# SvenGronauer/distributedTensorFlow

Hardware: AMD Instinct MI355X
Metric: images/sec (whole node) ResNet-50 synthetic ImageNet at 1/2/4/8 MI355X (higher is better)
Workload: dtype bf16; 1 GPU; model=resnet50, global_batch=1984, per_gpu_batch=1984, image_size=224, parallelism=dp1, impl=dtf, optimizer=momentum0.9+wd1e-4, lr 0.1*B/256 warmup500+cosine, backend=auto, native_ext=distributedtensorflow_amd/_lib/_dtf_hip.cpython-310-x86_64-linux-gnu.so

## Files before the change

### csrc/kernels/bindings.cpp

```cpp
#include <hip/hip_runtime.h>
#include <pybind11/pybind11.h>
#include <pybind11/stl.h>

#include <algorithm>
#include <stdexcept>
#include <string>
#include <vector>

#include "launch.h"

namespace py = pybind11;

namespace dlp {
struct Device { int32_t device_type; int32_t device_id; };
struct DataType { uint8_t code; uint8_t bits; uint16_t lanes; };
struct Tensor { void* data; Device device; int32_t ndim; DataType dtype; int64_t* shape;
                int64_t* strides; uint64_t byte_offset; };
struct Managed { Tensor t; void* ctx; void (*deleter)(Managed*); };
constexpr int32_t kROCM = 10;
struct Ctx { int64_t shape[1]; int64_t strides[1]; uintptr_t ptr; int device; bool opened; };
void deleter(Managed* m) {
  auto* c = static_cast<Ctx*>(m->ctx);
  if (c->opened) dtf_ipc_close(c->ptr, c->device);
  else dtf_ipc_free(c->ptr, c->device);
// ... 652 lines not shown
    check_launch("gemm_stream_bnb_dual");
  });
  m.def("gemm_set_group", &dtf_gemm_set_group);
  m.def("wgrad_get_pipe", &dtf_wgrad_get_pipe);
  m.def("lds_probe", [](int bytes, int blocks, uintptr_t errors, int spin, uintptr_t st) {
    dtf_lds_probe(bytes, blocks, P<int>(errors), spin, S(st));
    check_launch("lds_probe");
  });
  m.def("max_dynamic_lds", &dtf_max_dynamic_lds);

  m.def("ln_fwd", [](uintptr_t a, uintptr_t bias, uintptr_t res, uintptr_t gamma, uintptr_t beta,
                     uintptr_t y, uintptr_t s, uintptr_t mean, uintptr_t rstd, int M, int H,
                     float eps, float p_pre, uint32_t seed_pre, float p_post, uint32_t seed_post,
                     uintptr_t ids, uintptr_t tt, uintptr_t word, uintptr_t pos, uintptr_t type,
                     int S_, uintptr_t st) {
    dtf_ln_fwd(P<const bf16_t>(a), P<const float>(bias), P<const bf16_t>(res),
               P<const float>(gamma), P<const float>(beta), P<bf16_t>(y), P<bf16_t>(s),
               P<float>(mean), P<float>(rstd), M, H, eps, p_pre, seed_pre, p_post, seed_post,
               P<const int64_t>(ids), P<const int64_t>(tt), P<const bf16_t>(word),
               P<const bf16_t>(pos), P<const bf16_t>(type), S_, S(st));
    check_launch("ln_fwd");
  });
  m.def("ln_bwd_blocks", &dtf_ln_bwd_blocks);
  m.def("ln_bwd", [](uintptr_t dy, uintptr_t s, uintptr_t mean, uintptr_t rstd, uintptr_t gamma,
                     uintptr_t ds, uintptr_t da, uintptr_t part, uintptr_t dgamma,
                     uintptr_t dbeta, uintptr_t dbias, int M, int H, float p_pre,
                     uint32_t seed_pre, float p_post, uint32_t seed_post, uintptr_t st,
                     int accumulate) {
    dtf_ln_bwd(P<const bf16_t>(dy), P<const bf16_t>(s), P<const float>(mean),
               P<const float>(rstd), P<const float>(gamma), P<bf16_t>(ds), P<bf16_t>(da),
               P<float>(part), P<float>(dgamma), P<float>(dbeta), P<float>(dbias), M, H, p_pre,
               seed_pre, p_post, seed_post, S(st), accumulate);
    check_launch("ln_bwd");
  }, py::arg("dy"), py::arg("s"), py::arg("mean"), py::arg("rstd"), py::arg("gamma"),
     py::arg("ds"), py::arg("da"), py::arg("part"), py::arg("dgamma"), py::arg("dbeta"),
     py::arg("dbias"), py::arg("M"), py::arg("H"), py::arg("p_pre"), py::arg("seed_pre"),
     py::arg("p_post"), py::arg("seed_post"), py::arg("stream"), py::arg("accumulate") = 0);
  m.def("bias_gelu_fwd", [](uintptr_t a, uintptr_t bias, uintptr_t y, long M, int N,
                            uintptr_t st) {
    dtf_bias_gelu_fwd(P<const bf16_t>(a), P<const float>(bias), P<bf16_t>(y), M, N, S(st));
    check_launch("bias_gelu_fwd");
  });
  m.def("bias_gelu_bwd_blocks", &dtf_bias_gelu_bwd_blocks);
  m.def("bf16_col_sum_ws_floats", &dtf_bf16_col_sum_ws_floats);
  m.def("bf16_col_sum", [](uintptr_t x, int T, int N, uintptr_t ws, uintptr_t out, int accumulate,
                           uintptr_t stream) {
    dtf_bf16_col_sum(P<const bf16_t>(x), T, N, P<float>(ws), P<float>(out), accumulate, S(stream));
  });
  m.def("ln_set_wide", &dtf_ln_set_wide);
  m.def("conv1x1_bwd_ok", &dtf_conv1x1_bwd_ok);
  m.def("conv1x1_bwd_blocks", &dtf_conv1x1_bwd_blocks);
  m.def("conv1x1_bwd_set_grid", &dtf_conv1x1_bwd_set_grid);
  m.def("conv1x1_bwd_set_w16", &dtf_conv1x1_bwd_set_w16);
  m.def("conv1x1_bwd_lazy_ok", &dtf_conv1x1_bwd_lazy_ok);
  m.def("conv1x1_bwd_lazy_blocks", &dtf_conv1x1_bwd_lazy_blocks);
  m.def("conv1x1_bwd_lazy", [](uintptr_t dy3, uintptr_t x3, uintptr_t mask, uintptr_t cA,
                               uintptr_t cB, uintptr_t cC, uintptr_t wt, uintptr_t y, uintptr_t x,
                               uintptr_t mean, uintptr_t inv, uintptr_t sc, uintptr_t sh,
                               uintptr_t dy, uintptr_t wpart, uintptr_t bpart, int M, int C, int K,
                               uintptr_t w, uintptr_t stream) {
    dtf_conv1x1_bwd_lazy(P<bf16_t>(dy3), P<bf16_t>(x3), P<uint8_t>(mask), P<float>(cA),
                         P<float>(cB), P<float>(cC), P<bf16_t>(wt), P<bf16_t>(y), P<bf16_t>(x),
                         P<float>(mean), P<float>(inv), P<float>(sc), P<float>(sh), P<bf16_t>(dy),
                         P<float>(wpart), P<float>(bpart), M, C, K, P<bf16_t>(w), S(stream));
    check_launch("conv1x1_bwd_lazy");
  });
  m.def("conv1x1_bwd", [](uintptr_t dout, uintptr_t wt, uintptr_t y, uintptr_t x, uintptr_t mean,
                          uintptr_t inv, uintptr_t sc, uintptr_t sh, uintptr_t dy, uintptr_t wpart,
                          uintptr_t bpart, int M, int C, int K, uintptr_t stream) {
    dtf_conv1x1_bwd(P<bf16_t>(dout), P<bf16_t>(wt), P<bf16_t>(y), P<bf16_t>(x), P<float>(mean),
                    P<float>(inv), P<float>(sc), P<float>(sh), P<bf16_t>(dy), P<float>(wpart),
                    P<float>(bpart), M, C, K, S(stream));
    check_launch("conv1x1_bwd");
  });
  m.def("slab_reduce", [](uintptr_t ws, uintptr_t out, long n, int nsplit, int accumulate,
                          uintptr_t stream) {
    dtf_slab_reduce(P<const float>(ws), P<float>(out), n, nsplit, accumulate, S(stream));
  });
  m.def("bias_gelu_bwd", [](uintptr_t dy, uintptr_t a, uintptr_t bias, uintptr_t da,
                            uintptr_t part, uintptr_t dbias, int M, int N, uintptr_t st,
                            int accumulate) {
    dtf_bias_gelu_bwd(P<const bf16_t>(dy), P<const bf16_t>(a), P<const float>(bias),
                      P<bf16_t>(da), P<float>(part), P<float>(dbias), M, N, S(st), accumulate);
    check_launch("bias_gelu_bwd");
  }, py::arg("dy"), py::arg("a"), py::arg("bias"), py::arg("da"), py::arg("part"),
     py::arg("dbias"), py::arg("M"), py::arg("N"), py::arg("stream"), py::arg("accumulate") = 0);
  m.def("attn_fwd", [](uintptr_t qkv, uintptr_t mask, uintptr_t out, uintptr_t lse, int B, int S_,
                       int H, float scale, float p, uint32_t seed, uintptr_t st, uintptr_t keep) {
    dtf_attn_fwd(P<const bf16_t>(qkv), P<const float>(mask), P<bf16_t>(out), P<float>(lse), B,
                 S_, H, scale, p, seed, S(st), P<uint32_t>(keep));
    check_launch("attn_fwd");
  }, py::arg("qkv"), py::arg("mask"), py::arg("out"), py::arg("lse"), py::arg("B"), py::arg("S"),
     py::arg("H"), py::arg("scale"), py::arg("p"), py::arg("seed"), py::arg("st"),
     py::arg("keep") = 0);
  m.def("attn_keep_words", &dtf_attn_keep_words);
  m.def("attn_set_keep", &dtf_attn_set_keep);
  m.def("attn_bwd", [](uintptr_t qkv, uintptr_t mask, uintptr_t out, uintptr_t dout,
                       uintptr_t lse, uintptr_t delta, uintptr_t dqkv, int B, int S_, int H,
                       float scale, float p, uint32_t seed, uintptr_t st, uintptr_t colpart,
                       uintptr_t keep) {
    dtf_attn_bwd(P<const bf16_t>(qkv), P<const float>(mask), P<const bf16_t>(out),
                 P<const bf16_t>(dout), P<const float>(lse), P<float>(delta), P<bf16_t>(dqkv), B,
                 S_, H, scale, p, seed, S(st), P<float>(colpart), P<const uint32_t>(keep));
    check_launch("attn_bwd");
  }, py::arg("qkv"), py::arg("mask"), py::arg("out"), py::arg("dout"), py::arg("lse"),
     py::arg("delta"), py::arg("dqkv"), py::arg("B"), py::arg("S"), py::arg("H"),
// ... 38 lines not shown
```

### csrc/kernels/conv1x1_bwd.hip

```cpp
#include <stdexcept>
#include <string>

#include "launch.h"

namespace {

constexpr int kNB = 3;

typedef __attribute__((ext_vector_type(4))) short s4_t;
typedef __attribute__((address_space(3))) s4_t lds_s4_t;

template <int C_, int K_, int TM_, int NW_, bool LZ_ = false, bool RC_ = false>
struct Cfg {
  static constexpr int C = C_, K = K_, TM = TM_, NW = NW_;
  static constexpr bool LZ = LZ_, RC = RC_;
  static constexpr int T = NW * 64;
  static constexpr int NCB = C / 16;
  static constexpr int CPW = NCB >= NW ? NCB / NW : 1;
  static constexpr int WPC = NW / (NCB / CPW);
  static constexpr int MBW = TM / 16 / WPC;
  static constexpr int KS = K / 32;
  static constexpr int KBW = K / NW / 16;
  static constexpr int DO = TM * K;
  static constexpr int YT = TM * C;
  static constexpr int OT = (LZ && !RC) ? 2 * DO : DO;
  static constexpr int MB = LZ ? TM * K / 8 : 0;
  static constexpr int MI = MB / 1024;
  static constexpr int SLOT = OT + 2 * YT + MB / 2;
  static constexpr int DOI = OT * 2 / 1024;
  static constexpr int YI = YT * 2 / 1024;
  static constexpr int D = (DOI + 2 * YI) / NW;
  static constexpr int S = CPW * MBW;
  static constexpr int MCH = LZ ? TM * K / 8 / T : 0;
  static constexpr size_t LDS = (size_t)kNB * SLOT * 2 + (size_t)WPC * 2 * C * 4 + 4 * C * 4 +
                                (LZ ? (size_t)3 * K * 4 : 0);
  static_assert(!LZ || ((RC || ((TM * K / 8) % T == 0 && T % (K / 8) == 0)) && MB % 1024 == 0 &&
                        MI <= NW), "LZ transform split");
  static_assert(DOI % NW == 0 && (2 * YI) % NW == 0, "DMA split");
  static_assert(WPC * (NCB / CPW) == NW && MBW >= 1 && (TM % 32 == 0 || TM == 16), "wave split");
  static_assert(LDS <= 160 * 1024, "conv1x1_bwd LDS");
};

DTF_DEV int swz_o(int r) { return 2 * (r & 7) + ((r >> 3) & 1); }
template <int C>
DTF_DEV int swz_y(int r) { return C == 64 ? 2 * ((r >> 1) & 3) : 2 * (r & 7); }
template <int C>
DTF_DEV int swz_x(int r) { return C == 64 ? (r >> 1) & 7 : r & 15; }

template <int RP>
DTF_DEV int sidx(int r, int c, int s) { return r * RP + (((c >> 3) ^ s) << 3) + (c & 7); }

template <int RP, int C, bool DOUT>
DTF_DEV bf16x8_t tr8(const bf16_t* base, int row0, int col0, int lane) {
  const int i = lane & 15, g = lane >> 4;
  const int r = row0 + 4 * g + (i >> 2), c = col0 + 4 * (i & 3);
  const int s0 = DOUT ? swz_o(r) : swz_y<C>(r);
  const int s1 = DOUT ? swz_o(r + 16) : swz_y<C>(r + 16);
  const s4_t lo = __builtin_amdgcn_ds_read_tr16_b64_v4i16((lds_s4_t*)(base + sidx<RP>(r, c, s0)));
  const s4_t hi = __builtin_amdgcn_ds_read_tr16_b64_v4i16((lds_s4_t*)(base + sidx<RP>(r + 16, c, s1)));
  return (bf16x8_t){lo[0], lo[1], lo[2], lo[3], hi[0], hi[1], hi[2], hi[3]};
}

template <int RP, int C, bool DOUT>
DTF_DEV s4_t tr4(const bf16_t* base, int col0, int lane) {
  const int i = lane & 15, g = lane >> 4;
  const int r = 4 * g + (i >> 2), c = col0 + 4 * (i & 3);
  const int s0 = DOUT ? swz_o(r) : swz_y<C>(r);
  return __builtin_amdgcn_ds_read_tr16_b64_v4i16((lds_s4_t*)(base + sidx<RP>(r, c, s0)));
}

DTF_DEV f32x4_t mfma16(const bf16x8_t& a, const bf16x8_t& b, const f32x4_t& c) {
  return __builtin_amdgcn_mfma_f32_16x16x32_bf16(a, b, c, 0, 0, 0);
}

template <class F>
constexpr int RC_KBW() { return F::RC ? F::K / F::NW / 16 : 1; }

struct C1Args {
  const bf16_t* dout;
  const bf16_t* wt;
  const bf16_t* y;
  const bf16_t* x;
  const float* mean;
  const float* inv;
  const float* sc;
  const float* sh;
  bf16_t* dy;
  float* wpart;
  float* bpart;
  int M;
  const bf16_t* x3;
  const uint8_t* mask;
  const float* cA;
  const float* cB;
  const float* cC;
  const bf16_t* w;
};

template <class F>
__global__ void __launch_bounds__(F::T, 1) conv1x1_bwd_kernel(const C1Args g) {
  constexpr int C = F::C, K = F::K, TM = F::TM, NW = F::NW;
  constexpr int CPW = F::CPW, MBW = F::MBW, KS = F::KS, KBW = F::KBW, NCB = F::NCB;
  constexpr bool LZ = F::LZ;
  extern __shared__ __attribute__((aligned(16))) bf16_t lds[];
  float* sred = reinterpret_cast<float*>(lds + kNB * F::SLOT);
  float* sprm = sred + F::WPC * 2 * C;
  float* scoef = sprm + 4 * C;
  const int tid = threadIdx.x, lane = tid & 63;
  const int wave = __builtin_amdgcn_readfirstlane(tid >> 6);
  const int li = lane & 15, gq = lane >> 4;
  const int ntiles = g.M / TM;
  const int nmy = (ntiles - (int)blockIdx.x + (int)gridDim.x - 1) / (int)gridDim.x;
  const int cg = wave % (NCB / CPW), mw = wave / (NCB / CPW);

  bf16x8_t wf[CPW][KS];
#pragma unroll
  for (int j = 0; j < CPW; ++j)
#pragma unroll
    for (int ks = 0; ks < KS; ++ks)
      wf[j][ks] = *reinterpret_cast<const bf16x8_t*>(g.wt + ((cg * CPW + j) * 16 + li) * K +
                                                      ks * 32 + gq * 8);
  for (int t = tid; t < C; t += F::T) {
    sprm[t] = g.mean[t];
    sprm[C + t] = g.inv[t];
    sprm[2 * C + t] = g.sc[t];
    sprm[3 * C + t] = g.sh[t];
  }

  const uint32_t lds0 = lds_addr(lds);
  auto issue = [&](int i) {
    const bool live = !LZ || i < nmy;
    const long m0 = ((long)blockIdx.x + (long)(live ? i : 0) * gridDim.x) * TM;
    const i32x4_t ro = rsrc_quad(g.dout + m0 * K, (uint32_t)(F::DO * 2));
    const i32x4_t r3 = rsrc_quad(LZ ? g.x3 + m0 * K : g.dout, (uint32_t)(F::DO * 2));
    const i32x4_t ry = rsrc_quad(g.y + m0 * C, (uint32_t)(F::YT * 2));
    const i32x4_t rx = rsrc_quad(g.x + m0 * C, (uint32_t)(F::YT * 2));
    const uint32_t base = lds0 + (uint32_t)((i % kNB) * F::SLOT * 2);
    constexpr int OL = K / 8, YL = C / 8;
    constexpr int OI1 = F::DO * 2 / 1024;
#pragma unroll
    for (int j = 0; j < F::DOI / NW; ++j) {
      const int q = wave + NW * j;
      const int qq = q % OI1, e = qq * 64 + lane;
      const int r = e / OL, s = e % OL;
      const uint32_t off = live ? (uint32_t)((r * K + ((s ^ swz_o(r)) << 3)) * 2) : 0xFFFFFFF0u;
      dma16(q < OI1 ? ro : r3, base + (uint32_t)q * 1024u, off);
    }
#pragma unroll
    for (int j = 0; j < 2 * F::YI / NW; ++j) {
      const int q = wave + NW * j;
      const bool isx = q >= F::YI;
      const int qq = isx ? q - F::YI : q, e = qq * 64 + lane;
      const int r = e / YL, s = e % YL;
      const int sw = isx ? swz_x<C>(r) : swz_y<C>(r);
      const uint32_t off = live ? (uint32_t)((r * C + ((s ^ sw) << 3)) * 2) : 0xFFFFFFF0u;
      dma16(isx ? rx : ry, base + (uint32_t)(F::OT * 2 + q * 1024), off);
    }
    if constexpr (LZ) {
      if (wave < F::MI) {
        const i32x4_t rm = rsrc_quad(g.mask + m0 * (K / 8), (uint32_t)F::MB);
        dma16(rm, base + (uint32_t)((F::OT + 2 * F::YT) * 2 + wave * 1024),
              live ? (uint32_t)(wave * 1024 + lane * 16) : 0xFFFFFFF0u);
      }
    }
  };
  constexpr int MCH = F::MCH > 0 ? F::MCH : 1;
  if constexpr (LZ) {
    for (int t = tid; t < K; t += F::T) {
      scoef[t] = g.cA[t];
      scoef[K + t] = g.cB[t];
      scoef[2 * K + t] = g.cC[t];
    }
  }
  constexpr int KSC = C / 32;
  bf16x8_t wr[RC_KBW<F>()][KSC];
  float rca[RC_KBW<F>()][4], rcb[RC_KBW<F>()][4], rcc[RC_KBW<F>()][4];
  if constexpr (F::RC) {
#pragma unroll
    for (int kb = 0; kb < RC_KBW<F>(); ++kb) {
#pragma unroll
      for (int ks = 0; ks < KSC; ++ks)
        wr[kb][ks] = *reinterpret_cast<const bf16x8_t*>(
            g.w + (long)(wave * (K / NW) + kb * 16 + li) * C + ks * 32 + gq * 8);
      const int k0 = wave * (K / NW) + kb * 16 + 4 * gq;
#pragma unroll
      for (int r = 0; r < 4; ++r) {
        rca[kb][r] = g.cA[k0 + r];
        rcb[kb][r] = g.cB[k0 + r];
        rcc[kb][r] = g.cC[k0 + r];
      }
    }
  }

  f32x4_t aw[KBW][NCB];
#pragma unroll
  for (int a = 0; a < KBW; ++a)
#pragma unroll
    for (int b = 0; b < NCB; ++b) aw[a][b] = (f32x4_t){0.f, 0.f, 0.f, 0.f};
  float s1[CPW][4], s2[CPW][4];
#pragma unroll
  for (int j = 0; j < CPW; ++j)
#pragma unroll
    for (int e = 0; e < 4; ++e) s1[j][e] = s2[j][e] = 0.f;

  constexpr int D = F::D, S = F::S;
  if constexpr (LZ) {
    issue(0);
    issue(1);
  } else {
    issue(0);
    if (nmy > 1) issue(1);
  }
  for (int i = 0; i < nmy; ++i) {
    if constexpr (LZ) {
      if (wave < F::MI) {
        if (i == 0) wait_vm<D + 1>();
        else if (i == 1) wait_vm<D + 1 + S>();
        else wait_vm<D + 1 + 2 * S>();
      } else {
        if (i == 0) wait_vm<D>();
        else if (i == 1) wait_vm<D + S>();
        else wait_vm<D + 2 * S>();
      }
    } else {
      const bool more = i + 1 < nmy;
      if (i == 0) { if (more) wait_vm<D>(); else wait_vm<0>(); }
      else if (i == 1) { if (more) wait_vm<D + S>(); else wait_vm<S>(); }
      else { if (more) wait_vm<D + 2 * S>(); else wait_vm<2 * S>(); }
    }
    asm volatile("s_waitcnt lgkmcnt(0)" ::: "memory");
    raw_barrier();
    if constexpr (LZ) {
      issue(i + 2);
    } else {
      if (i + 2 < nmy) issue(i + 2);
    }
    bf16_t* const slot = lds + (i % kNB) * F::SLOT;
    if constexpr (LZ && F::RC) {
      int lx = lane;
      asm volatile("" : "+v"(lx));
      const int xi = lx & 15, xq = lx >> 4;
      const uint8_t* msk = reinterpret_cast<const uint8_t*>(slot + F::OT + 2 * F::YT);
#pragma unroll
      for (int mb = 0; mb < TM / 16; ++mb) {
        const int m = mb * 16 + xi;
        bf16x8_t yb[KSC];
#pragma unroll
        for (int ks = 0; ks < KSC; ++ks)
          yb[ks] = *reinterpret_cast<const bf16x8_t*>(slot + F::OT + sidx<C>(m, ks * 32 + xq * 8, swz_y<C>(m)));
#pragma unroll
        for (int kb = 0; kb < RC_KBW<F>(); ++kb) {
          f32x4_t a = (f32x4_t){0.f, 0.f, 0.f, 0.f};
#pragma unroll
          for (int ks = 0; ks < KSC; ++ks) a = mfma16(wr[kb][ks], yb[ks], a);
          const int k0 = wave * (K / NW) + kb * 16 + 4 * xq;
          const int o = sidx<K>(m, k0, swz_o(m));
          const uint2 d = *reinterpret_cast<const uint2*>(slot + o);
          const uint32_t mbits = (uint32_t)msk[m * (K / 8) + (k0 >> 3)] >> (k0 & 7);
          const float* ca = rca[kb];
          const float* cb = rcb[kb];
          const float* cc = rcc[kb];
          const float gv[4] = {__builtin_bit_cast(float, d.x << 16), __builtin_bit_cast(float, d.x & 0xffff0000u),
                               __builtin_bit_cast(float, d.y << 16), __builtin_bit_cast(float, d.y & 0xffff0000u)};
          float ov[4];
#pragma unroll
          for (int r = 0; r < 4; ++r) {
            const float xv = bf2f(f2bf(a[r]));
            const float dz = (mbits >> r) & 1u ? gv[r] : 0.f;
            ov[r] = bn_bwd_dx(ca[r], dz, cb[r], xv, cc[r]);
          }
          *reinterpret_cast<uint2*>(slot + o) = make_uint2(pack2(ov[0], ov[1]), pack2(ov[2], ov[3]));
        }
      }
      asm volatile("s_waitcnt lgkmcnt(0)" ::: "memory");
      raw_barrier();
    } else if constexpr (LZ) {
      int tt = tid;
      asm volatile("" : "+v"(tt));
      const int lch = tt % (K / 8), lrow = tt / (K / 8);
#pragma unroll
      for (int k = 0; k < MCH; ++k) {
        const int r = lrow + k * (F::T / (K / 8));
        const int o = sidx<K>(r, lch * 8, swz_o(r));
        float gv[8], xv[8], ov[8];
        unpack8(*reinterpret_cast<const uint4*>(slot + o), gv);
        unpack8(*reinterpret_cast<const uint4*>(slot + F::DO + o), xv);
        const uint32_t mb = reinterpret_cast<const uint8_t*>(slot + F::OT + 2 * F::YT)[r * (K / 8) + lch];
        float ca[8], cb[8], cc[8];
        *reinterpret_cast<float4*>(ca) = *reinterpret_cast<const float4*>(scoef + lch * 8);
        *reinterpret_cast<float4*>(ca + 4) = *reinterpret_cast<const float4*>(scoef + lch * 8 + 4);
        *reinterpret_cast<float4*>(cb) = *reinterpret_cast<const float4*>(scoef + K + lch * 8);
        *reinterpret_cast<float4*>(cb + 4) = *reinterpret_cast<const float4*>(scoef + K + lch * 8 + 4);
        *reinterpret_cast<float4*>(cc) = *reinterpret_cast<const float4*>(scoef + 2 * K + lch * 8);
        *reinterpret_cast<float4*>(cc + 4) = *reinterpret_cast<const float4*>(scoef + 2 * K + lch * 8 + 4);
#pragma unroll
        for (int e = 0; e < 8; ++e) {
          const float dz = (mb >> e) & 1u ? gv[e] : 0.f;
          ov[e] = bn_bwd_dx(ca[e], dz, cb[e], xv[e], cc[e]);
        }
        *reinterpret_cast<uint4*>(slot + o) = pack8(ov);
      }
      asm volatile("s_waitcnt lgkmcnt(0)" ::: "memory");
      raw_barrier();
    }
    const bf16_t* sO = slot;
    const bf16_t* sY = sO + F::OT;
    const bf16_t* sX = sY + F::YT;
    int ln = lane;
    asm volatile("" : "+v"(ln));
    const int li = ln & 15, gq = ln >> 4;

    f32x4_t ad[CPW][MBW];
#pragma unroll
    for (int j = 0; j < CPW; ++j)
#pragma unroll
      for (int f = 0; f < MBW; ++f) ad[j][f] = (f32x4_t){0.f, 0.f, 0.f, 0.f};
#pragma unroll
    for (int ks = 0; ks < KS; ++ks) {
#pragma unroll
      for (int f = 0; f < MBW; ++f) {
        const int m = (mw * MBW + f) * 16 + li;
        const bf16x8_t b = *reinterpret_cast<const bf16x8_t*>(sO + sidx<K>(m, ks * 32 + gq * 8, swz_o(m)));
#pragma unroll
        for (int j = 0; j < CPW; ++j) ad[j][f] = mfma16(wf[j][ks], b, ad[j][f]);
      }
    }
    if constexpr (TM == 16) {
      s4_t fa[KBW];
#pragma unroll
      for (int kb = 0; kb < KBW; ++kb) fa[kb] = tr4<K, C, true>(sO, wave * (K / NW) + kb * 16, ln);
#pragma unroll
      for (int cb = 0; cb < NCB; ++cb) {
        const s4_t fb = tr4<C, C, false>(sY, cb * 16, ln);
#pragma unroll
        for (int kb = 0; kb < KBW; ++kb)
          aw[kb][cb] = __builtin_amdgcn_mfma_f32_16x16x16bf16_1k(fa[kb], fb, aw[kb][cb], 0, 0, 0);
      }
    }
#pragma unroll
    for (int ms = 0; ms < TM / 32; ++ms) {
      bf16x8_t fa[KBW];
#pragma unroll
      for (int kb = 0; kb < KBW; ++kb) fa[kb] = tr8<K, C, true>(sO, 32 * ms, wave * (K / NW) + kb * 16, ln);
#pragma unroll
      for (int cb = 0; cb < NCB; ++cb) {
        const bf16x8_t fb = tr8<C, C, false>(sY, 32 * ms, cb * 16, ln);
#pragma unroll
        for (int kb = 0; kb < KBW; ++kb) aw[kb][cb] = mfma16(fa[kb], fb, aw[kb][cb]);
      }
    }
    const long m0 = ((long)blockIdx.x + (long)i * gridDim.x) * TM;
#pragma unroll
    for (int j = 0; j < CPW; ++j) {
      const int c0 = (cg * CPW + j) * 16 + 4 * gq;
      float mu[4], is[4], sc[4], sh[4];
#pragma unroll
      for (int e = 0; e < 4; ++e) {
        mu[e] = sprm[c0 + e];
        is[e] = sprm[C + c0 + e];
        sc[e] = sprm[2 * C + c0 + e];
        sh[e] = sprm[3 * C + c0 + e];
      }
#pragma unroll
      for (int f = 0; f < MBW; ++f) {
        const int m = (mw * MBW + f) * 16 + li;
        const uint2 pk = make_uint2(pack2(ad[j][f][0], ad[j][f][1]), pack2(ad[j][f][2], ad[j][f][3]));
        *reinterpret_cast<uint2*>(g.dy + (m0 + m) * C + c0) = pk;
        const uint2 xr = *reinterpret_cast<const uint2*>(sX + sidx<C>(m, c0, swz_x<C>(m)));
        const float gd[4] = {__builtin_bit_cast(float, pk.x << 16), __builtin_bit_cast(float, pk.x & 0xffff0000u),
                             __builtin_bit_cast(float, pk.y << 16), __builtin_bit_cast(float, pk.y & 0xffff0000u)};
        const float xv[4] = {__builtin_bit_cast(float, xr.x << 16), __builtin_bit_cast(float, xr.x & 0xffff0000u),
                             __builtin_bit_cast(float, xr.y << 16), __builtin_bit_cast(float, xr.y & 0xffff0000u)};
#pragma unroll
        for (int e = 0; e < 4; ++e) {
          const float dz = __builtin_fmaf(xv[e], sc[e], sh[e]) > 0.f ? gd[e] : 0.f;
          s1[j][e] += dz;
          s2[j][e] += dz * (xv[e] - mu[e]) * is[e];
        }
      }
    }
  }
  DTF_WAIT_VM(0);
  asm volatile("s_waitcnt lgkmcnt(0)" ::: "memory");
  raw_barrier();

#pragma unroll
  for (int j = 0; j < CPW; ++j)
#pragma unroll
    for (int e = 0; e < 4; ++e) {
#pragma unroll
      for (int o = 1; o < 16; o <<= 1) {
        s1[j][e] += __shfl_xor(s1[j][e], o, 64);
        s2[j][e] += __shfl_xor(s2[j][e], o, 64);
      }
    }
  if (li == 0) {
#pragma unroll
    for (int j = 0; j < CPW; ++j)
#pragma unroll
      for (int e = 0; e < 4; ++e) {
        const int c = (cg * CPW + j) * 16 + 4 * gq + e;
        sred[(mw * 2 + 0) * C + c] = s1[j][e];
        sred[(mw * 2 + 1) * C + c] = s2[j][e];
      }
  }
  __syncthreads();
  for (int t = tid; t < 2 * C; t += F::T) {
    const int which = t / C, col = t % C;
    float v = 0.f;
#pragma unroll
    for (int w = 0; w < F::WPC; ++w) v += sred[(w * 2 + which) * C + col];
    g.bpart[((long)blockIdx.x * 2 + which) * C + col] = v;
  }
  float* wp = g.wpart + (long)blockIdx.x * K * C;
#pragma unroll
  for (int kb = 0; kb < KBW; ++kb)
#pragma unroll
    for (int cb = 0; cb < NCB; ++cb)
#pragma unroll
      for (int r = 0; r < 4; ++r)
        wp[(wave * (K / NW) + kb * 16 + 4 * gq + r) * C + cb * 16 + li] = aw[kb][cb][r];
}

typedef Cfg<64, 256, 64, 8> CfgS0;
typedef Cfg<64, 256, 64, 16> CfgS0W;
typedef Cfg<128, 512, 32, 8> CfgS1;
typedef Cfg<64, 256, 64, 8, true, true> CfgS0L;
typedef Cfg<64, 256, 64, 16, true, true> CfgS0LW;
typedef Cfg<128, 512, 16, 8, true> CfgS1L;

int g_c1_grid = 0;
int g_c1_w16 = 0;

int c1_tm(int C) { return C == 64 ? CfgS0::TM : CfgS1::TM; }

int c1_blocks_tm(int M, int TM) {
  static int cus = 0;
  if (!cus) {
    int dev = 0;
    HIP_CHECK(hipGetDevice(&dev));
    HIP_CHECK(hipDeviceGetAttribute(&cus, hipDeviceAttributeMultiprocessorCount, dev));
  }
  const int want = g_c1_grid > 0 ? g_c1_grid : cus;
  const int ntiles = M / TM;
  return ntiles < want ? ntiles : want;
}
int c1_blocks(int M, int C) { return c1_blocks_tm(M, c1_tm(C)); }

template <class F>
void launch_c1(const C1Args& g, hipStream_t st) {
  static bool attr = false;
  if (!attr) {
    HIP_CHECK(hipFuncSetAttribute((const void*)conv1x1_bwd_kernel<F>,
                                  hipFuncAttributeMaxDynamicSharedMemorySize, (int)F::LDS));
    attr = true;
  }
  hipLaunchKernelGGL(conv1x1_bwd_kernel<F>, dim3(c1_blocks_tm(g.M, F::TM)), dim3(F::T), F::LDS, st,
                     g);
}

}

bool dtf_conv1x1_bwd_ok(int M, int C, int K) {
  return ((C == 64 && K == 256) || (C == 128 && K == 512)) && M > 0 && M % c1_tm(C) == 0;
}

int dtf_conv1x1_bwd_blocks(int M, int C) {
  if (!dtf_conv1x1_bwd_ok(M, C, 4 * C)) throw std::runtime_error("conv1x1_bwd: shape");
  return c1_blocks(M, C);
}

void dtf_conv1x1_bwd_set_grid(int n) { g_c1_grid = n; }
void dtf_conv1x1_bwd_set_w16(int v) { g_c1_w16 = v; }

void dtf_conv1x1_bwd(const bf16_t* dout, const bf16_t* wt, const bf16_t* y, const bf16_t* x,
                     const float* mean, const float* inv, const float* sc, const float* sh,
                     bf16_t* dy, float* wpart, float* bpart, int M, int C, int K, hipStream_t st) {
  if (!dtf_conv1x1_bwd_ok(M, C, K))
    throw std::runtime_error("conv1x1_bwd: (C, K) in {(64, 256), (128, 512)}, M % tile == 0");
  const void* ptrs[] = {dout, wt, y, x, mean, inv, sc, sh, dy, wpart, bpart};
  for (const void* p : ptrs)
    if (!p || (reinterpret_cast<uintptr_t>(p) & 15))
      throw std::runtime_error("conv1x1_bwd: null or misaligned operand");
  C1Args g{dout, wt, y, x, mean, inv, sc, sh, dy, wpart, bpart, M};
  if (C == 64) {
    if (g_c1_w16) launch_c1<CfgS0W>(g, st);
    else launch_c1<CfgS0>(g, st);
  } else {
    launch_c1<CfgS1>(g, st);
  }
}

bool dtf_conv1x1_bwd_lazy_ok(int M, int C, int K) {
  if (M <= 0) return false;
  if (C == CfgS0L::C && K == CfgS0L::K) return M % CfgS0L::TM == 0;
  if (C == CfgS1L::C && K == CfgS1L::K) return M % CfgS1L::TM == 0;
  return false;
}
int dtf_conv1x1_bwd_lazy_blocks(int M, int C) {
  if (!dtf_conv1x1_bwd_lazy_ok(M, C, 4 * C)) throw std::runtime_error("conv1x1_bwd_lazy: shape");
  return c1_blocks_tm(M, C == 64 ? CfgS0L::TM : CfgS1L::TM);
}
void dtf_conv1x1_bwd_lazy(const bf16_t* dy3, const bf16_t* x3, const uint8_t* mask,
                          const float* cA, const float* cB, const float* cC, const bf16_t* wt,
                          const bf16_t* y, const bf16_t* x, const float* mean, const float* inv,
                          const float* sc, const float* sh, bf16_t* dy, float* wpart,
                          float* bpart, int M, int C, int K, const bf16_t* w, hipStream_t st) {
  if (!dtf_conv1x1_bwd_lazy_ok(M, C, K))
    throw std::runtime_error("conv1x1_bwd_lazy: (C, K) in {(64, 256), (128, 512)}, M % tile == 0");
  const void* ptrs[] = {dy3, x3, mask, cA, cB, cC, wt, y, x, mean, inv, sc, sh, dy, wpart, bpart, w};
  for (const void* p : ptrs)
    if (!p || (reinterpret_cast<uintptr_t>(p) & 15))
      throw std::runtime_error("conv1x1_bwd_lazy: null or misaligned operand");
  C1Args g{dy3, wt, y, x, mean, inv, sc, sh, dy, wpart, bpart, M, x3, mask, cA, cB, cC, w};
  if (C == 64) {
    if (g_c1_w16) launch_c1<CfgS0LW>(g, st);
    else launch_c1<CfgS0L>(g, st);
  } else {
    launch_c1<CfgS1L>(g, st);
  }
}
```

### csrc/kernels/launch.h

```cpp
#pragma once
#include <string>
#include <vector>

#include "common.h"

#define DTF_MAX_TAPS 64

struct TapTable {
  int n;
  int dh[DTF_MAX_TAPS];
  int dw[DTF_MAX_TAPS];
};

struct TapTableW {
  int n;
  int dh[DTF_MAX_TAPS];
  int dw[DTF_MAX_TAPS];
};

struct ConvGeom {
  int N, H, W, C;
  int P, Q;
  int sh, sw;
  int Kout;
// ... 88 lines not shown
                           const float* cAp, const float* cBp, const float* cCp, bf16_t* dxp,
                           long M, int C, hipStream_t st);

void dtf_conv_set_small_k(int mode);
void dtf_conv_set_dma_mode(int mode);
void dtf_conv_set_halo(int on);
void dtf_conv_set_halo_strips(int v);
void dtf_conv_set_halo_freg(int v);
void dtf_conv_set_halo_stages(int v);
void dtf_conv_set_bnl_probe(int v);
void dtf_conv_set_stem_halo(int v);
void dtf_conv_set_halo_bnb(int v);
int dtf_conv_stats_rows(long M, int Kout, int C, int taps, int W);
void dtf_conv_set_gemm(int v);
int dtf_conv_tile_rows(const ConvGeom& g, const TapTable& taps, int bnb);
void dtf_conv_set_nt(int v);
bool dtf_conv_bnl_ok(const ConvGeom& g, const TapTable& taps);
void dtf_conv_igemm(const bf16_t* X, const bf16_t* Wt, bf16_t* Y, const ConvGeom& g_in,
                    const TapTable& taps, int bk, float* stats, const BnBwdEpi& bnb,
                    hipStream_t st);
bool dtf_conv_igemm_grouped(const bf16_t* X, bf16_t* Y, const ConvGeom& g0, int ncls,
                            const bf16_t* const* wts, const int* oh0, const int* ow0,
                            const int* kpad, const std::vector<std::vector<int>>& dh,
                            const std::vector<std::vector<int>>& dw, const BnBwdEpi& bnb,
                            const int* row0, hipStream_t st);
void dtf_filter_transpose(const WtJobs& jobs, hipStream_t st);

void dtf_wgrad_set_dma_mode(int mode);
void dtf_wgrad_set_pp(int v);
void dtf_wgrad_set_dense(int v);
void dtf_wgrad_set_deep(int v);
void dtf_wgrad_set_direct(int v);
void dtf_wgrad_set_pipe(int p);
int dtf_wgrad_get_pipe();
void dtf_wgrad_set_halo(int v);
void dtf_wgrad_set_stem(int v);
int dtf_conv_wgrad_halo_splits(int N, int H, int W, int C, int P, int Q, int Kout, int sh, int sw,
                               const TapTableW& taps);
int dtf_conv_wgrad_splits(long M, int Kout, int TC, long ws_cap, int taps);
void dtf_conv_wgrad(const bf16_t* X, const bf16_t* dY, float* dW, float* ws, WgradGeom g,
                    const TapTableW& taps, int splits, int tr_mode, int accumulate, hipStream_t st);
void dtf_slab_reduce(const float* ws, float* out, long n, int nsplit, int accumulate,
                     hipStream_t st);
int dtf_wgrad_stem_dz_splits(int N);
void dtf_conv_wgrad_stem_dz(const bf16_t* X, const bf16_t* dp, const uint8_t* arg,
                            const bf16_t* xbn, const float* ca, const float* cb, const float* cc,
                            const float* fsc, const float* fsh, float* dW, float* ws, int N,
                            int accumulate, hipStream_t st);

bool dtf_conv1x1_bwd_ok(int M, int C, int K);
int dtf_conv1x1_bwd_blocks(int M, int C);
void dtf_conv1x1_bwd_set_grid(int n);
void dtf_conv1x1_bwd_set_w16(int v);
void dtf_conv1x1_bwd(const bf16_t* dout, const bf16_t* wt, const bf16_t* y, const bf16_t* x,
                     const float* mean, const float* inv, const float* sc, const float* sh,
                     bf16_t* dy, float* wpart, float* bpart, int M, int C, int K, hipStream_t st);
bool dtf_conv1x1_bwd_lazy_ok(int M, int C, int K);
int dtf_conv1x1_bwd_lazy_blocks(int M, int C);
void dtf_conv1x1_bwd_lazy(const bf16_t* dy3, const bf16_t* x3, const uint8_t* mask, const float* cA,
                          const float* cB, const float* cC, const bf16_t* wt, const bf16_t* y,
                          const bf16_t* x, const float* mean, const float* inv, const float* sc,
                          const float* sh, bf16_t* dy, float* wpart, float* bpart, int M, int C,
                          int K, const bf16_t* w, hipStream_t st);

void dtf_gemm_set_variant(int v);
void dtf_gemm_set_stream(int v);
void dtf_gemm_set_pp2(int v);
void dtf_gemm_set_pp2_strided(int v);
int dtf_gemm_get_pp2();
void dtf_gemm_set_nt(int v);
void dtf_gemm_set_dbg(int v);
void dtf_gemm_set_group(int gm);
int dtf_gemm_conv_part_images(int N, int H, int W, int C, int P, int Q);
void dtf_gemm_conv(const bf16_t* X, const bf16_t* Wt, bf16_t* Y, int N, int H, int W, int C, int P,
                   int Q, int sh, int sw, int Kout, int ntaps, const int* dh, const int* dw, int Ho,
                   int Wo, int osh, int osw, int oh0, int ow0, float* stats, const bf16_t* Cin,
                   const bf16_t* acc_src, const uint8_t* acc_mask, hipStream_t st);
void dtf_gemm_nt_gelu_bwd(const bf16_t* A, const bf16_t* B, bf16_t* C, int M, int N, int K, int lda,
                          int ldb, const bf16_t* gelu_a, const float* gelu_b, float* colsum,
                          hipStream_t st);
void dtf_gemm_nt_bias_gelu(const bf16_t* A, const bf16_t* B, bf16_t* Z, bf16_t* H, int M, int N,
                           int K, int lda, int ldb, const float* bias, hipStream_t st);
bool dtf_gemm_pp2_ok(int M, int N, int K, int lda, int ldb);
int dtf_gemm_tile_rows(int M);
void dtf_gemm_nt(const bf16_t* A, const bf16_t* B, bf16_t* C, int M, int N, int K, int lda, int ldb,
                 int ldc, const float* bias, const bf16_t* Cin, int relu, float* stats,
                 hipStream_t st, const bf16_t* acc_src, const uint8_t* acc_mask);

bool dtf_gemm_stream_ok(int M, int N, int K, int lda, int ldb, int ldc);
void dtf_gemm_stream(const bf16_t* A, const bf16_t* B, bf16_t* C, int M, int N, int K, int lda,
                     int ldb, int ldc, const bf16_t* Cin, float* stats, const bf16_t* acc_src,
                     const uint8_t* acc_mask, int nt, hipStream_t st);
void dtf_gemm_stream_bnb(const bf16_t* A, const bf16_t* B, bf16_t* C, int M, int N, int K, int lda,
                         int ldb, int ldc, const bf16_t* Cin, const bf16_t* acc_src,
                         const uint8_t* acc_mask, const bf16_t* bx, const float* bmean,
                         const float* binv, const float* bsc, const float* bsh,
                         const uint8_t* bmask, int kind, float* part, int nt, hipStream_t st,
                         const bf16_t* y2, const bf16_t* w3, int k3);
void dtf_gemm_stream_bnb_dual(const bf16_t* A, const bf16_t* B, bf16_t* C, int M, int N, int K,
                              int lda, int ldb, int ldc, const bf16_t* Cin, const bf16_t* acc_src,
                              const uint8_t* acc_mask, const bf16_t* bx, const float* bmean,
                              const float* binv, const uint8_t* bmask, float* part,
                              const bf16_t* bxp, const float* bmeanp, const float* binvp,
                              float* part_p, hipStream_t st);
void dtf_gemm_stream_pre(const bf16_t* X, const bf16_t* B, bf16_t* C, int M, int N, int K,
                         const float* pre_sc, const float* pre_sh, bf16_t* y, float* stats,
// ... 172 lines not shown
```

### distributedtensorflow_amd/ops/native.py

```python
from __future__ import annotations

import os

import torch

from .records import BnDeferred as _BnDeferred
from .records import GradSlot as _GradSlot
from .records import LazyBnDx as _LazyBnDx
from .records import LazyStemDz as _LazyStemDz
from .records import MaskedGrad as _MaskedGrad
from .records import Recompute as _Recompute
from .records import end_step as end_step
from .reference import resolve_padding, space_to_depth_operands

try:
    from .._lib import _dtf_hip as _K
except ImportError as e:
    raise ImportError(
        "distributedtensorflow_amd HIP extension (_lib/_dtf_hip*.so) is not built; run "
        "`python -m distributedtensorflow_amd._build` (hipcc --offload-arch=gfx950). "
        f"Original error: {e}") from e

_BF16 = torch.bfloat16
_DENSE_IMPL = os.environ.get("DTF_DENSE", "native")


def _store_nt(v):
    _K.conv_set_nt(v & 1)
    _K.gemm_set_nt((v >> 1) & 1)
    _K.bn_set_nt(7 if v & 4 else 0)


_ENV_KNOBS = (
    ("DTF_WGRAD_MODE", _K.wgrad_set_dma_mode, ""),
    ("DTF_WGRAD_PP", _K.wgrad_set_pp, "ping-pong wgrad: 0 off, n: split-K target of n rounds"),
    ("DTF_WGRAD_DENSE", _K.wgrad_set_dense, "ping-pong wgrad's decode-free one-tap form: 0 off"),
    ("DTF_WGRAD_PIPE", _K.wgrad_set_pipe, ""),
    ("DTF_CONV_DMA", _K.conv_set_dma_mode, ""),
    ("DTF_CONV_HALO", _K.conv_set_halo, ""),
    ("DTF_WGRAD_HALO", _K.wgrad_set_halo, ""),
    ("DTF_CONV_STEM_HALO", _K.conv_set_stem_halo, ""),
    ("DTF_CONV_HALO_STRIPS", _K.conv_set_halo_strips,
     "bit f: two strips per block for halo family f"),
    ("DTF_CONV_HALO_FREG", _K.conv_set_halo_freg,
     "bit f: halo family f streams its filter via VGPRs"),
    ("DTF_CONV_SMALL_K", _K.conv_set_small_k, ""),
    ("DTF_GEMM_STREAM", _K.gemm_set_stream,
     "row-streaming GEMM for output-heavy shapes (default on)"),
    ("DTF_C1_W16", _K.conv1x1_bwd_set_w16,
     "stage-0 fused c3 backward as 16-wave blocks (default 0)"),
    ("DTF_GEMM_GROUP_M", _K.gemm_set_group, "grouped tile order of the dense GEMMs (0: N fastest)"),
    ("DTF_BN_GRID_CAP", _K.bn_set_grid_cap,
     "BN row-sweep grid cap override (2048 = round-2 grids)"),
    ("DTF_BN_STATS_BLOCKS", _K.bn_set_stats_blocks, "BN reduce-pass block target (1024 = round-2)"),
    ("DTF_GEMM_PP2", _K.gemm_set_pp2, "round-5 persistent GEMM: bit 0 gemm_nt (default), 1 convs"),
    ("DTF_STORE_NT", _store_nt, "non-temporal output stores: bit 0 conv, 1 GEMM, 2 BN"),
)
for _name, _setter, _ in _ENV_KNOBS:
    if os.environ.get(_name):
        _setter(int(os.environ[_name]))


def _st():
    return torch.cuda.current_stream().cuda_stream


def _p(t):
    return 0 if t is None else t.data_ptr()


def _pair(v):
    return (v, v) if isinstance(v, int) else tuple(v)


def _bf16_weight(w: torch.Tensor) -> torch.Tensor:
    s = getattr(w, "_dtf_shadow", None)
    if s is not None and s.dtype == _BF16:
        return s
    return w.detach().to(_BF16)


_DIRECT_GRAD = os.environ.get("DTF_DIRECT_GRAD", "1") == "1"


def _direct_grad(p):
    if not _DIRECT_GRAD or p is None or not getattr(p, "_dtf_flat", False):
        return None
    g = p.grad
    if g is None or g.dtype != torch.float32 or not g.is_contiguous():
        return None
    return g




def enable_timing_probe(name, value=1):
    setter = {"bnl": _K.conv_set_bnl_probe, "stream_bnb": _K.gemm_stream_set_bnb_probe}[name]
    setter(int(value))


def _grad_ready(p):
    cb = getattr(p, "_dtf_grad_ready", None)
    if cb is not None:
# ... 1664 lines not shown
```

Baseline: 17100 images/sec.

## Pipeline stage-0 lazy conv1x1 backward: transform next tile while computing current

Splits the stage-0 lazy fused conv1x1 backward loop into transform and compute lambdas. A new PIPE config transforms tile i+1 while compute runs on tile i, with the two halves of the waves swapping phase order, which removes one barrier per tile. The aim is to overlap the VALU-heavy BN-dx transform with the MFMA work. It also drops the compiler-opaque asm pins on lane indices (HOIST), and adds probe variants that are compiled only behind a build flag. It becomes the default path, so the LDS slot reuse and barrier ordering carry race risk.

Result: no change. 17120 images/sec, median of 2 (+0.1%).

```diff
diff --git a/csrc/kernels/bindings.cpp b/csrc/kernels/bindings.cpp
--- a/csrc/kernels/bindings.cpp
+++ b/csrc/kernels/bindings.cpp
@@ -728,6 +728,8 @@
   m.def("conv1x1_bwd_blocks", &dtf_conv1x1_bwd_blocks);
   m.def("conv1x1_bwd_set_grid", &dtf_conv1x1_bwd_set_grid);
   m.def("conv1x1_bwd_set_w16", &dtf_conv1x1_bwd_set_w16);
+  m.def("conv1x1_bwd_set_pipe", &dtf_conv1x1_bwd_set_pipe);
+  m.def("conv1x1_bwd_set_probe", &dtf_conv1x1_bwd_set_probe);
   m.def("conv1x1_bwd_lazy_ok", &dtf_conv1x1_bwd_lazy_ok);
   m.def("conv1x1_bwd_lazy_blocks", &dtf_conv1x1_bwd_lazy_blocks);
   m.def("conv1x1_bwd_lazy", [](uintptr_t dy3, uintptr_t x3, uintptr_t mask, uintptr_t cA,
diff --git a/csrc/kernels/conv1x1_bwd.hip b/csrc/kernels/conv1x1_bwd.hip
--- a/csrc/kernels/conv1x1_bwd.hip
+++ b/csrc/kernels/conv1x1_bwd.hip
@@ -9,11 +9,13 @@
 
 typedef __attribute__((ext_vector_type(4))) short s4_t;
 typedef __attribute__((address_space(3))) s4_t lds_s4_t;
-
-template <int C_, int K_, int TM_, int NW_, bool LZ_ = false, bool RC_ = false>
+typedef uint32_t u32x2_t __attribute__((ext_vector_type(2)));
+
+template <int C_, int K_, int TM_, int NW_, bool LZ_ = false, bool RC_ = false,
+          bool PIPE_ = false, bool HOIST_ = false>
 struct Cfg {
   static constexpr int C = C_, K = K_, TM = TM_, NW = NW_;
-  static constexpr bool LZ = LZ_, RC = RC_;
+  static constexpr bool LZ = LZ_, RC = RC_, PIPE = PIPE_, HOIST = HOIST_;
   static constexpr int T = NW * 64;
   static constexpr int NCB = C / 16;
   static constexpr int CPW = NCB >= NW ? NCB / NW : 1;
@@ -39,6 +41,7 @@
   static_assert(DOI % NW == 0 && (2 * YI) % NW == 0, "DMA split");
   static_assert(WPC * (NCB / CPW) == NW && MBW >= 1 && (TM % 32 == 0 || TM == 16), "wave split");
   static_assert(LDS <= 160 * 1024, "conv1x1_bwd LDS");
+  static_assert(!PIPE || (LZ && NW % 2 == 0), "PIPE: the LZ forms, two halves");
 };
 
 DTF_DEV int swz_o(int r) { return 2 * (r & 7) + ((r >> 3) & 1); }
@@ -97,7 +100,7 @@
   const bf16_t* w;
 };
 
-template <class F>
+template <class F, int PROBE = 0>
 __global__ void __launch_bounds__(F::T, 1) conv1x1_bwd_kernel(const C1Args g) {
   constexpr int C = F::C, K = F::K, TM = F::TM, NW = F::NW;
   constexpr int CPW = F::CPW, MBW = F::MBW, KS = F::KS, KBW = F::KBW, NCB = F::NCB;
@@ -204,41 +207,11 @@
     for (int e = 0; e < 4; ++e) s1[j][e] = s2[j][e] = 0.f;
 
   constexpr int D = F::D, S = F::S;
-  if constexpr (LZ) {
-    issue(0);
-    issue(1);
-  } else {
-    issue(0);
-    if (nmy > 1) issue(1);
-  }
-  for (int i = 0; i < nmy; ++i) {
-    if constexpr (LZ) {
-      if (wave < F::MI) {
-        if (i == 0) wait_vm<D + 1>();
-        else if (i == 1) wait_vm<D + 1 + S>();
-        else wait_vm<D + 1 + 2 * S>();
-      } else {
-        if (i == 0) wait_vm<D>();
-        else if (i == 1) wait_vm<D + S>();
-        else wait_vm<D + 2 * S>();
-      }
-    } else {
-      const bool more = i + 1 < nmy;
-      if (i == 0) { if (more) wait_vm<D>(); else wait_vm<0>(); }
-      else if (i == 1) { if (more) wait_vm<D + S>(); else wait_vm<S>(); }
-      else { if (more) wait_vm<D + 2 * S>(); else wait_vm<2 * S>(); }
-    }
-    asm volatile("s_waitcnt lgkmcnt(0)" ::: "memory");
-    raw_barrier();
-    if constexpr (LZ) {
-      issue(i + 2);
-    } else {
-      if (i + 2 < nmy) issue(i + 2);
-    }
+  auto transform = [&](int i) {
     bf16_t* const slot = lds + (i % kNB) * F::SLOT;
-    if constexpr (LZ && F::RC) {
+    if constexpr (LZ && F::RC && !(PROBE & 1)) {
       int lx = lane;
-      asm volatile("" : "+v"(lx));
+      if constexpr (!F::HOIST) asm volatile("" : "+v"(lx));
       const int xi = lx & 15, xq = lx >> 4;
       const uint8_t* msk = reinterpret_cast<const uint8_t*>(slot + F::OT + 2 * F::YT);
 #pragma unroll
@@ -272,11 +245,9 @@
           *reinterpret_cast<uint2*>(slot + o) = make_uint2(pack2(ov[0], ov[1]), pack2(ov[2], ov[3]));
         }
       }
-      asm volatile("s_waitcnt lgkmcnt(0)" ::: "memory");
-      raw_barrier();
-    } else if constexpr (LZ) {
+    } else if constexpr (LZ && !(PROBE & 1)) {
       int tt = tid;
-      asm volatile("" : "+v"(tt));
+      if constexpr (!F::HOIST) asm volatile("" : "+v"(tt));
       const int lch = tt % (K / 8), lrow = tt / (K / 8);
 #pragma unroll
       for (int k = 0; k < MCH; ++k) {
@@ -300,14 +271,15 @@
         }
         *reinterpret_cast<uint4*>(slot + o) = pack8(ov);
       }
-      asm volatile("s_waitcnt lgkmcnt(0)" ::: "memory");
-      raw_barrier();
-    }
+    }
+  };
+  auto compute = [&](int i) {
+    const bf16_t* const slot = lds + (i % kNB) * F::SLOT;
     const bf16_t* sO = slot;
     const bf16_t* sY = sO + F::OT;
     const bf16_t* sX = sY + F::YT;
     int ln = lane;
-    asm volatile("" : "+v"(ln));
+    if constexpr (!F::HOIST) asm volatile("" : "+v"(ln));
     const int li = ln & 15, gq = ln >> 4;
 
     f32x4_t ad[CPW][MBW];
@@ -316,7 +288,7 @@
 #pragma unroll
       for (int f = 0; f < MBW; ++f) ad[j][f] = (f32x4_t){0.f, 0.f, 0.f, 0.f};
 #pragma unroll
-    for (int ks = 0; ks < KS; ++ks) {
+    for (int ks = 0; ks < ((PROBE & 4) ? 0 : KS); ++ks) {
 #pragma unroll
       for (int f = 0; f < MBW; ++f) {
         const int m = (mw * MBW + f) * 16 + li;
@@ -325,7 +297,7 @@
         for (int j = 0; j < CPW; ++j) ad[j][f] = mfma16(wf[j][ks], b, ad[j][f]);
       }
     }
-    if constexpr (TM == 16) {
+    if constexpr (TM == 16 && !(PROBE & 2)) {
       s4_t fa[KBW];
 #pragma unroll
       for (int kb = 0; kb < KBW; ++kb) fa[kb] = tr4<K, C, true>(sO, wave * (K / NW) + kb * 16, ln);
@@ -338,7 +310,7 @@
       }
     }
 #pragma unroll
-    for (int ms = 0; ms < TM / 32; ++ms) {
+    for (int ms = 0; ms < ((PROBE & 2) ? 0 : TM / 32); ++ms) {
       bf16x8_t fa[KBW];
 #pragma unroll
       for (int kb = 0; kb < KBW; ++kb) fa[kb] = tr8<K, C, true>(sO, 32 * ms, wave * (K / NW) + kb * 16, ln);
@@ -365,7 +337,13 @@
       for (int f = 0; f < MBW; ++f) {
         const int m = (mw * MBW + f) * 16 + li;
         const uint2 pk = make_uint2(pack2(ad[j][f][0], ad[j][f][1]), pack2(ad[j][f][2], ad[j][f][3]));
-        *reinterpret_cast<uint2*>(g.dy + (m0 + m) * C + c0) = pk;
+        if constexpr (PROBE & 8) {
+          __builtin_amdgcn_raw_buffer_store_b64((u32x2_t){pk.x, pk.y}, buffer_rsrc(g.dy, 0u),
+                                                (int)(((m0 + m) * C + c0) * 2), 0, 0);
+        } else {
+          *reinterpret_cast<uint2*>(g.dy + (m0 + m) * C + c0) = pk;
+        }
+        if constexpr (PROBE & 4) continue;
         const uint2 xr = *reinterpret_cast<const uint2*>(sX + sidx<C>(m, c0, swz_x<C>(m)));
         const float gd[4] = {__builtin_bit_cast(float, pk.x << 16), __builtin_bit_cast(float, pk.x & 0xffff0000u),
                              __builtin_bit_cast(float, pk.y << 16), __builtin_bit_cast(float, pk.y & 0xffff0000u)};
@@ -379,6 +357,71 @@
         }
       }
     }
+  };
+
+  if constexpr (LZ && F::PIPE) {
+    issue(0);
+    issue(1);
+    if (wave < F::MI) wait_vm<D + 1>();
+    else wait_vm<D>();
+    asm volatile("s_waitcnt lgkmcnt(0)" ::: "memory");
+    raw_barrier();
+    transform(0);
+    const bool tfirst = wave < NW / 2;
+    for (int i = 0; i < nmy; ++i) {
+      if (i == 0) wait_vm<0>();
+      else wait_vm<S>();
+      asm volatile("s_waitcnt lgkmcnt(0)" ::: "memory");
+      raw_barrier();
+      issue(i + 2);
+#pragma nounroll
+      for (int ph = 0; ph < 2; ++ph) {
+        if ((ph == 0) == tfirst) {
+          if (i + 1 < nmy) transform(i + 1);
+        } else {
+          compute(i);
+        }
+      }
+    }
+  } else {
+    if constexpr (LZ) {
+      issue(0);
+      issue(1);
+    } else {
+      issue(0);
+      if (nmy > 1) issue(1);
+    }
+    for (int i = 0; i < nmy; ++i) {
+      if constexpr (LZ) {
+        if (wave < F::MI) {
+          if (i == 0) wait_vm<D + 1>();
+          else if (i == 1) wait_vm<D + 1 + S>();
+          else wait_vm<D + 1 + 2 * S>();
+        } else {
+          if (i == 0) wait_vm<D>();
+          else if (i == 1) wait_vm<D + S>();
+          else wait_vm<D + 2 * S>();
+        }
+      } else {
+        const bool more = i + 1 < nmy;
+        if (i == 0) { if (more) wait_vm<D>(); else wait_vm<0>(); }
+        else if (i == 1) { if (more) wait_vm<D + S>(); else wait_vm<S>(); }
+        else { if (more) wait_vm<D + 2 * S>(); else wait_vm<2 * S>(); }
+      }
+      asm volatile("s_waitcnt lgkmcnt(0)" ::: "memory");
+      raw_barrier();
+      if constexpr (LZ) {
+        issue(i + 2);
+      } else {
+        if (i + 2 < nmy) issue(i + 2);
+      }
+      if constexpr (LZ && !(PROBE & 1)) {
+        transform(i);
+        asm volatile("s_waitcnt lgkmcnt(0)" ::: "memory");
+        raw_barrier();
+      }
+      compute(i);
+    }
   }
   DTF_WAIT_VM(0);
   asm volatile("s_waitcnt lgkmcnt(0)" ::: "memory");
@@ -422,15 +465,21 @@
         wp[(wave * (K / NW) + kb * 16 + 4 * gq + r) * C + cb * 16 + li] = aw[kb][cb][r];
 }
 
+
 typedef Cfg<64, 256, 64, 8> CfgS0;
 typedef Cfg<64, 256, 64, 16> CfgS0W;
 typedef Cfg<128, 512, 32, 8> CfgS1;
 typedef Cfg<64, 256, 64, 8, true, true> CfgS0L;
+typedef Cfg<64, 256, 64, 8, true, true, true, true> CfgS0LP;
 typedef Cfg<64, 256, 64, 16, true, true> CfgS0LW;
 typedef Cfg<128, 512, 16, 8, true> CfgS1L;
 
 int g_c1_grid = 0;
 int g_c1_w16 = 0;
+int g_c1_pipe = 1;
+#ifdef DTF_PROBES
+int g_c1_probe = 0;
+#endif
 
 int c1_tm(int C) { return C == 64 ? CfgS0::TM : CfgS1::TM; }
 
@@ -447,16 +496,31 @@
 }
 int c1_blocks(int M, int C) { return c1_blocks_tm(M, c1_tm(C)); }
 
+template <class F, int PROBE>
+void launch_c1p(const C1Args& g, hipStream_t st) {
+  static bool attr = false;
+  if (!attr) {
+    HIP_CHECK(hipFuncSetAttribute((const void*)conv1x1_bwd_kernel<F, PROBE>,
+                                  hipFuncAttributeMaxDynamicSharedMemorySize, (int)F::LDS));
+    attr = true;
+  }
+  hipLaunchKernelGGL((conv1x1_bwd_kernel<F, PROBE>), dim3(c1_blocks_tm(g.M, F::TM)), dim3(F::T),
+                     F::LDS, st, g);
+}
+
 template <class F>
 void launch_c1(const C1Args& g, hipStream_t st) {
-  static bool attr = false;
-  if (!attr) {
-    HIP_CHECK(hipFuncSetAttribute((const void*)conv1x1_bwd_kernel<F>,
-                                  hipFuncAttributeMaxDynamicSharedMemorySize, (int)F::LDS));
-    attr = true;
-  }
-  hipLaunchKernelGGL(conv1x1_bwd_kernel<F>, dim3(c1_blocks_tm(g.M, F::TM)), dim3(F::T), F::LDS, st,
-                     g);
+#ifdef DTF_PROBES
+  switch (g_c1_probe) {
+    case 1: launch_c1p<F, 1>(g, st); return;
+    case 2: launch_c1p<F, 2>(g, st); return;
+    case 4: launch_c1p<F, 4>(g, st); return;
+    case 8: launch_c1p<F, 8>(g, st); return;
+    case 15: launch_c1p<F, 15>(g, st); return;
+    default: break;
+  }
+#endif
+  launch_c1p<F, 0>(g, st);
 }
 
 }
@@ -472,6 +536,18 @@
 
 void dtf_conv1x1_bwd_set_grid(int n) { g_c1_grid = n; }
 void dtf_conv1x1_bwd_set_w16(int v) { g_c1_w16 = v; }
+void dtf_conv1x1_bwd_set_pipe(int v) { g_c1_pipe = v; }
+
+void dtf_conv1x1_bwd_set_probe(int v) {
+#ifdef DTF_PROBES
+  if (v != 0 && v != 1 && v != 2 && v != 4 && v != 8 && v != 15)
+    throw std::runtime_error("conv1x1_bwd_set_probe: one of 0, 1, 2, 4, 8, 15");
+  g_c1_probe = v;
+#else
+  if (v) throw std::runtime_error("conv1x1_bwd_set_probe: a timing probe with wrong results; "
+                                  "build with DTF_HIP_EXTRA_FLAGS=-DDTF_PROBES (tools only)");
+#endif
+}
 
 void dtf_conv1x1_bwd(const bf16_t* dout, const bf16_t* wt, const bf16_t* y, const bf16_t* x,
                      const float* mean, const float* inv, const float* sc, const float* sh,
@@ -515,6 +591,7 @@
   C1Args g{dy3, wt, y, x, mean, inv, sc, sh, dy, wpart, bpart, M, x3, mask, cA, cB, cC, w};
   if (C == 64) {
     if (g_c1_w16) launch_c1<CfgS0LW>(g, st);
+    else if (g_c1_pipe) launch_c1<CfgS0LP>(g, st);
     else launch_c1<CfgS0L>(g, st);
   } else {
     launch_c1<CfgS1L>(g, st);
diff --git a/csrc/kernels/launch.h b/csrc/kernels/launch.h
--- a/csrc/kernels/launch.h
+++ b/csrc/kernels/launch.h
@@ -164,6 +164,8 @@
 int dtf_conv1x1_bwd_blocks(int M, int C);
 void dtf_conv1x1_bwd_set_grid(int n);
 void dtf_conv1x1_bwd_set_w16(int v);
+void dtf_conv1x1_bwd_set_pipe(int v);
+void dtf_conv1x1_bwd_set_probe(int v);
 void dtf_conv1x1_bwd(const bf16_t* dout, const bf16_t* wt, const bf16_t* y, const bf16_t* x,
                      const float* mean, const float* inv, const float* sc, const float* sh,
                      bf16_t* dy, float* wpart, float* bpart, int M, int C, int K, hipStream_t st);
diff --git a/distributedtensorflow_amd/ops/native.py b/distributedtensorflow_amd/ops/native.py
--- a/distributedtensorflow_amd/ops/native.py
+++ b/distributedtensorflow_amd/ops/native.py
@@ -49,6 +49,8 @@
      "row-streaming GEMM for output-heavy shapes (default on)"),
     ("DTF_C1_W16", _K.conv1x1_bwd_set_w16,
      "stage-0 fused c3 backward as 16-wave blocks (default 0)"),
+    ("DTF_C1_PIPE", _K.conv1x1_bwd_set_pipe,
+     "stage-0 lazy fused c3 backward: transform one tile ahead of the MFMA phases (default 1)"),
     ("DTF_GEMM_GROUP_M", _K.gemm_set_group, "grouped tile order of the dense GEMMs (0: N fastest)"),
     ("DTF_BN_GRID_CAP", _K.bn_set_grid_cap,
      "BN row-sweep grid cap override (2048 = round-2 grids)"),
```
